# tusen-ai/MV2D

Hardware: AMD Instinct MI355X
Metric: multi-view samples/sec (6-cam frames) through the MV2D RoI-head hot path (higher is better)
Workload: dtype f16x3: every operand an fp16 hi + lo pair, three MFMAs per product, fp32 accumulation (fp32-class, index-exact route; the lo halves of the key / value rows are STORED as e4m3 bytes); 1 GPU; cfg2_s: MV2D-S head, 6 views 1408x512; global_batch=384, streams_per_gpu=4, samples_per_launch=16, pe_sine_branch=folded into a per-(weights, geometry) table, FLOPs not counted, parallelism=dp1, hipgraph=True

## Files before the change

mv2d_amd/csrc/xattn_fused.hip:

```cpp
#include "xattn_walk.h"
#include <stdlib.h>
#ifndef MV2D_XF_QB_DEFAULT
#define MV2D_XF_QB_DEFAULT 8
#endif

#ifdef MV2D_XF_TRACE
__device__ long long g_xf_trace[32];
#define XF_STAMP(i) do { if (blockIdx.x == MV2D_XF_TRACE && threadIdx.x == 0) g_xf_trace[i] = (long long)__builtin_amdgcn_s_memtime(); } while (0)
#else
#define XF_STAMP(i) do {} while (0)
#endif

namespace {

constexpr int WAVE_LDS = 16384;

template <int XLO, int QB>
__global__ __launch_bounds__(64 * QB, 2) void xattn_fused_kernel(const float* __restrict__ q, const uint4* __restrict__ WA_hi, const uint4* __restrict__ WA_lo,
                                                                const uint4* __restrict__ WB_hi, const uint4* __restrict__ WB_lo, const float* __restrict__ bv,
                                                                const unsigned short* __restrict__ Xk, const unsigned short* __restrict__ Xv,
                                                                const unsigned short* __restrict__ Xk_lo, const unsigned short* __restrict__ Xv_lo,
                                                                const int* __restrict__ row_ptr, const int* __restrict__ col_idx, float* __restrict__ ctx,
                                                                int R, int empty_nan, const int* __restrict__ order, int nblk) {
    constexpr int SMEM = QB * WAVE_LDS + QB * 512 + QB * HEADS * 4 + 3 * QB * 4;
    __shared__ __attribute__((aligned(16))) unsigned char smem[SMEM];
    const int tid = threadIdx.x, lane = tid & 63, wave = tid >> 6, n = lane & 15, g = lane >> 4;
    float* lsum = reinterpret_cast<float*>(smem + QB * WAVE_LDS + QB * 512);
    int* rq = reinterpret_cast<int*>(smem + QB * WAVE_LDS + QB * 512 + QB * HEADS * 4);
    int* rbeg = rq + QB;
    int* rend = rq + 2 * QB;
    const int blk = xcd_chunked(blockIdx.x, nblk);
    const int slot0 = (int)((long long)blk * R / nblk), nq = (int)((long long)(blk + 1) * R / nblk) - slot0;
    if (nq <= 0) return;
    XF_STAMP(0);
    if (tid < QB) {
        const int s = slot0 + min(tid, nq - 1);
        const int r_ = order ? order[s] : s;
        rq[tid] = r_;
        rbeg[tid] = row_ptr[r_];
        rend[tid] = row_ptr[r_ + 1];
    }
    __syncthreads();
    XF_STAMP(1);
    const int beg = rbeg[wave], end = rend[wave];
    const int ntile = wave < nq ? (end - beg + 15) >> 4 : 0;
    int idx_next = ntile > 0 ? col_idx[min(beg + n, end - 1)] : 0;
    typedef XattnWalk<XLO, false> Walk;
    Walk walk(Xk, Xv, Xk_lo, Xv_lo, lane, beg, end, reinterpret_cast<uint4*>(smem + wave * WAVE_LDS), reinterpret_cast<uint4*>(smem + wave * WAVE_LDS) + 512,
           reinterpret_cast<float*>(smem + QB * WAVE_LDS) + wave * 128);
    typename Walk::KRows k0;
    for (int h = wave; h < HEADS; h += QB) {
        const int r = rq[n & (QB - 1)];
        const float* qp = q + (long long)r * C + 32 * h + 8 * g;
        const float4 q0 = *reinterpret_cast<const float4*>(qp), q1 = *reinterpret_cast<const float4*>(qp + 4);
        const uint4* wh = WA_hi + (long long)h * 16 * 64 + lane;
        const uint4* wl = WA_lo + (long long)h * 16 * 64 + lane;
        uint4* qt = reinterpret_cast<uint4*>(smem + (n & (QB - 1)) * WAVE_LDS) + h * 64;
        u32x4 wa_h[16], wa_l[16];
#pragma unroll
        for (int t = 0; t < 16; ++t) {
            wa_h[t] = *reinterpret_cast<const u32x4*>(wh + t * 64);
            wa_l[t] = *reinterpret_cast<const u32x4*>(wl + t * 64);
        }
        __builtin_amdgcn_sched_barrier(0);
        XF_STAMP(20);
        Frag bh, bl;
        split8(q0, q1, bh, bl);
#pragma unroll
        for (int u = 0; u < 8; ++u) {
            if (u == 1) XF_STAMP(21);
            if (u == 4) XF_STAMP(22);
            f32x4_t a[2];
#pragma unroll
            for (int k = 0; k < 2; ++k) {
                f32x4_t c = {0.f, 0.f, 0.f, 0.f};
                c = mfma_q16_16x16x32(wa_l[2 * u + k], bh.v, c);
                c = mfma_q16_16x16x32(wa_h[2 * u + k], bl.v, c);
                c = mfma_q16_16x16x32(wa_h[2 * u + k], bh.v, c);
                a[k] = c;
            }
            Frag hi, lo;
            split8_k16(make_float4(a[0][0], a[0][1], a[0][2], a[0][3]), make_float4(a[1][0], a[1][1], a[1][2], a[1][3]), hi, lo);
            if (n < QB) {
                qt[u * 8 + g * 2] = hi.u;
                qt[u * 8 + g * 2 + 1] = lo.u;
            }
            if (u == (XLO ? 5 : 3) && h == wave && ntile > 0) walk.request_k(idx_next, k0);
        }
    }
    XF_STAMP(23);
    asm volatile("s_waitcnt lgkmcnt(0)" ::: "memory");
    __builtin_amdgcn_s_barrier();
    XF_STAMP(2);
    {
        const uint4* qp = reinterpret_cast<const uint4*>(smem + wave * WAVE_LDS) + (n & 7) * 64 + g * 2 + (n >> 3);
#pragma unroll
        for (int s = 0; s < 8; ++s) walk.qa[s].u = qp[s * 8];
    }
    walk.reset();
    if (ntile > 0) walk.stage_k(k0);
#pragma nounroll
    for (int tt = 0; tt < ntile; ++tt) {
        const int myidx = idx_next;
        if (tt + 1 < ntile) idx_next = col_idx[min(beg + 16 * (tt + 1) + n, end - 1)];
        typename Walk::VRows v;
        walk.gather(myidx, tt > 0, v);
        XF_STAMP(3 + 2 * min(tt, 5));
        walk.compute(tt, v);
        XF_STAMP(4 + 2 * min(tt, 5));
    }
    walk.row_sums();
    if (n == 0 && g < 2) {
#pragma unroll
        for (int i = 0; i < 4; ++i) lsum[wave * HEADS + 4 * g + i] = walk.l_run[i];
    }
    walk.store_z(reinterpret_cast<float*>(smem + wave * WAVE_LDS));
    XF_STAMP(15);
    __syncthreads();
    XF_STAMP(16);
    for (int h = wave; h < HEADS; h += QB) {
        const int j = n & (QB - 1);
        const float* zp = reinterpret_cast<const float*>(smem + j * WAVE_LDS) + h * C + 8 * g;
        const float rl = __builtin_amdgcn_rcpf(lsum[j * HEADS + h]);
        const uint4* wh = WB_hi + (long long)h * 16 * 64 + lane;
        const uint4* wl = WB_lo + (long long)h * 16 * 64 + lane;
        f32x4_t acc[2] = {{0.f, 0.f, 0.f, 0.f}, {0.f, 0.f, 0.f, 0.f}};
        u32x4 wb_h[16], wb_l[16];
#pragma unroll
        for (int t = 0; t < 16; ++t) {
            wb_h[t] = *reinterpret_cast<const u32x4*>(wh + t * 64);
            wb_l[t] = *reinterpret_cast<const u32x4*>(wl + t * 64);
        }
        int rr_[4], rp0_[4], rp1_[4];
#pragma unroll
        for (int i = 0; i < 4; ++i) {
            rr_[i] = rq[(4 * g + i) & (QB - 1)];
            rp0_[i] = rbeg[(4 * g + i) & (QB - 1)];
            rp1_[i] = rend[(4 * g + i) & (QB - 1)];
        }
        const float bv0 = bv[32 * h + n], bv1 = bv[32 * h + 16 + n];
        __builtin_amdgcn_sched_barrier(0);
#pragma unroll
        for (int s = 0; s < 8; ++s) {
            float4 x0 = *reinterpret_cast<const float4*>(zp + 32 * s);
            float4 x1 = *reinterpret_cast<const float4*>(zp + 32 * s + 4);
            x0 = make_float4(x0.x * rl, x0.y * rl, x0.z * rl, x0.w * rl);
            x1 = make_float4(x1.x * rl, x1.y * rl, x1.z * rl, x1.w * rl);
            Frag ah, al;
            split8(x0, x1, ah, al);
#pragma unroll
            for (int nt = 0; nt < 2; ++nt) {
                acc[nt] = mfma_q16_16x16x32(al.v, wb_h[s * 2 + nt], acc[nt]);
                acc[nt] = mfma_q16_16x16x32(ah.v, wb_l[s * 2 + nt], acc[nt]);
                acc[nt] = mfma_q16_16x16x32(ah.v, wb_h[s * 2 + nt], acc[nt]);
            }
        }
        if (4 * g < QB) {
#pragma unroll
            for (int i = 0; i < 4; ++i) {
                const int js = 4 * g + i;
                if (js < nq) {
                    const int rr = rr_[i];
                    const bool empty = rp1_[i] <= rp0_[i];
#pragma unroll
                    for (int nt = 0; nt < 2; ++nt) {
                        const int col = 32 * h + 16 * nt + n;
                        float v = acc[nt][i] + (nt ? bv1 : bv0);
                        if (empty) v = empty_nan ? __uint_as_float(0x7fc00000u) : 0.f;
                        ctx[(long long)rr * C + col] = v;
                    }
                }
            }
        }
    }
    XF_STAMP(17);
}

}

#ifdef MV2D_XF_TRACE
extern "C" int mv2d_xf_trace_read(long long* host, int n) { return hipMemcpyFromSymbol(host, HIP_SYMBOL(g_xf_trace), n * sizeof(long long)) == hipSuccess ? 0 : -2; }
#endif

extern "C" int mv2d_xattn_fused_fwd(const float* q, const void* WA_hi, const void* WA_lo, const void* WB_hi, const void* WB_lo, const float* bv,
                                    const void* Xk, const void* Xv, const void* Xk_lo, const void* Xv_lo, const int* row_ptr, const int* col_idx,
                                    float* ctx, int R, int empty_nan, const int* order, int lo_fmt, void* stream) {
    MV2D_CHECK_ARG(lo_fmt == 0 || (lo_fmt == 1 && Xk_lo), "mv2d_xattn_fused_fwd: lo_fmt is 0 (key16 lo rows) or 1 (e4m3 lo rows; needs the lo rows)");
    MV2D_CHECK_ARG(q && WA_hi && WA_lo && WB_hi && WB_lo && bv && Xk && Xv && row_ptr && col_idx && ctx && R >= 0, "mv2d_xattn_fused_fwd: bad args");
    MV2D_CHECK_ARG((Xk_lo == nullptr) == (Xv_lo == nullptr), "mv2d_xattn_fused_fwd: Xk_lo and Xv_lo come together");
    MV2D_CHECK_ARG(((uintptr_t)q & 15) == 0 && ((uintptr_t)WA_hi & 15) == 0 && ((uintptr_t)WA_lo & 15) == 0 && ((uintptr_t)WB_hi & 15) == 0 &&
                       ((uintptr_t)WB_lo & 15) == 0 && ((uintptr_t)Xk & 15) == 0 && ((uintptr_t)Xv & 15) == 0 && ((uintptr_t)Xk_lo & 15) == 0 &&
                       ((uintptr_t)Xv_lo & 15) == 0, "mv2d_xattn_fused_fwd: operands must be 16-byte aligned");
    if (R == 0) return MV2D_OK;
    static int n_cu = 0;
    if (n_cu == 0) {
        hipDeviceProp_t prop;
        int dev = 0;
        n_cu = (hipGetDevice(&dev) == hipSuccess && hipGetDeviceProperties(&prop, dev) == hipSuccess && prop.multiProcessorCount > 0) ? prop.multiProcessorCount : 256;
    }
    static const int qb_env = [] { const char* e = getenv("MV2D_XF_QB"); return e ? atoi(e) : 0; }();
    const int QB = qb_env == 4 || qb_env == 8 ? qb_env : MV2D_XF_QB_DEFAULT;
    const int slots = n_cu * (QB == 4 ? 2 : 1);
    int nblk = (R + QB - 1) / QB;
    if (nblk > slots) {
        const int up = (nblk + slots - 1) / slots * slots;
        if ((long long)up * (QB / 2) <= R) nblk = up;
    } else {
        const int spread = R / 2 < n_cu ? R / 2 : n_cu;
        if (spread > nblk) nblk = spread;
    }
    const dim3 grid(nblk), block(64 * QB);
#define MV2D_XF(XLO_, QB_) hipLaunchKernelGGL((xattn_fused_kernel<XLO_, QB_>), grid, block, 0, (hipStream_t)stream, q, (const uint4*)WA_hi, (const uint4*)WA_lo, \
                                              (const uint4*)WB_hi, (const uint4*)WB_lo, bv, (const unsigned short*)Xk, (const unsigned short*)Xv,                     \
                                              (const unsigned short*)Xk_lo, (const unsigned short*)Xv_lo, row_ptr, col_idx, ctx, R, empty_nan, order, nblk)
    if (Xk_lo && lo_fmt == 1) { if (QB == 4) MV2D_XF(2, 4); else MV2D_XF(2, 8); }
    else if (Xk_lo) { if (QB == 4) MV2D_XF(1, 4); else MV2D_XF(1, 8); }
    else { if (QB == 4) MV2D_XF(0, 4); else MV2D_XF(0, 8); }
#undef MV2D_XF
    MV2D_LAUNCH_CHECK();
    return MV2D_OK;
}
```

mv2d_amd/csrc/xattn_walk.h:

```cpp
#pragma once
#include "common.h"
#include <type_traits>

namespace {

constexpr int C = 256, HEADS = 8;
constexpr float LOG2E = 1.4426950408889634f;

typedef q16x8_t q16x8;
union Frag { uint4 u; q16x8 v; };
typedef unsigned int u32x4 __attribute__((ext_vector_type(4)));
typedef unsigned int u32x2 __attribute__((ext_vector_type(2)));

__device__ __forceinline__ void split8(const float4& x0, const float4& x1, Frag& hi, Frag& lo) {
    const float f[8] = {x0.x, x0.y, x0.z, x0.w, x1.x, x1.y, x1.z, x1.w};
    unsigned int h[4], l[4];
#pragma unroll
    for (int i = 0; i < 4; ++i) split_q16x2(f[2 * i], f[2 * i + 1], h[i], l[i]);
    hi.u = make_uint4(h[0], h[1], h[2], h[3]);
    lo.u = make_uint4(l[0], l[1], l[2], l[3]);
}
__device__ __forceinline__ void split8_k16(const float4& x0, const float4& x1, Frag& hi, Frag& lo) {
    const float f[8] = {x0.x, x0.y, x0.z, x0.w, x1.x, x1.y, x1.z, x1.w};
    unsigned int h[4], l[4];
#pragma unroll
    for (int i = 0; i < 4; ++i) split_k16x2(f[2 * i], f[2 * i + 1], h[i], l[i]);
    hi.u = make_uint4(h[0], h[1], h[2], h[3]);
    lo.u = make_uint4(l[0], l[1], l[2], l[3]);
}

__device__ __forceinline__ unsigned int lo_pair(unsigned int a, unsigned int b) { return __builtin_amdgcn_perm(b, a, 0x05040100u); }
__device__ __forceinline__ unsigned int hi_pair(unsigned int a, unsigned int b) { return __builtin_amdgcn_perm(b, a, 0x07060302u); }

#define XATTN_DPP(v, ctrl) __uint_as_float((unsigned)__builtin_amdgcn_update_dpp(0, (int)__float_as_uint(v), ctrl, 0xF, 0xF, true))
__device__ __forceinline__ float row16_max(float v) {
    v = fmaxf(v, XATTN_DPP(v, 0xB1));
    v = fmaxf(v, XATTN_DPP(v, 0x4E));
    v = fmaxf(v, XATTN_DPP(v, 0x141));
    v = fmaxf(v, XATTN_DPP(v, 0x140));
    return v;
}

template <int XLO, bool DBG>
struct XattnWalk {
    typedef std::conditional_t<XLO == 2, u32x2, u32x4> lo_t;
    struct KRows { u32x4 hi[8]; lo_t lo[XLO ? 8 : 1]; };
    struct VRows { u32x4 hi[4][2]; lo_t lo[XLO ? 4 : 1][2]; };

    const unsigned short *Xk, *Xv, *Xk_lo, *Xv_lo;
    int lane, n, g, beg, end;
    uint4 *kt, *kt2;
    float* pl;
    float* dbg_logits;
    long long dbg_stride;
    Frag qa[8];
    float m_run[4], l_run[4];
    f32x4_t Z[16];

    __device__ __forceinline__ XattnWalk(const unsigned short* Xk_, const unsigned short* Xv_, const unsigned short* Xk_lo_, const unsigned short* Xv_lo_,
                                         int lane_, int beg_, int end_, uint4* kt_, uint4* kt2_, float* pl_, float* dbg_logits_ = nullptr,
                                         long long dbg_stride_ = 0)
        : Xk(Xk_), Xv(Xv_), Xk_lo(Xk_lo_), Xv_lo(Xv_lo_), lane(lane_), n(lane_ & 15), g(lane_ >> 4), beg(beg_), end(end_), kt(kt_), kt2(kt2_), pl(pl_),
          dbg_logits(dbg_logits_), dbg_stride(dbg_stride_) {}

    __device__ __forceinline__ void reset() {
#pragma unroll
        for (int i = 0; i < 4; ++i) { m_run[i] = -INFINITY; l_run[i] = 0.f; }
#pragma unroll
        for (int u = 0; u < 16; ++u) Z[u] = f32x4_t{0.f, 0.f, 0.f, 0.f};
    }

    __device__ __forceinline__ void load_v(const unsigned short* V_, int myidx, u32x4 (&dst)[4][2]) const {
#pragma unroll
        for (int e = 0; e < 4; ++e) {
            const unsigned int vidx = (unsigned int)__shfl(myidx, 4 * g + e, 64);
            const char* vp = reinterpret_cast<const char*>(V_) + ((vidx << 9) + 16u * (unsigned)n);
            dst[e][0] = *reinterpret_cast<const u32x4*>(vp);
            dst[e][1] = *reinterpret_cast<const u32x4*>(vp + 256);
        }
    }
    __device__ __forceinline__ void load_k(const unsigned short* K_, int myidx, u32x4 (&dst)[8]) const {
#pragma unroll
        for (int i = 0; i < 8; ++i) {
            const unsigned int ridx = (unsigned int)__shfl(myidx, 2 * i + (lane >> 5), 64);
            dst[i] = *reinterpret_cast<const u32x4*>(reinterpret_cast<const char*>(K_) + ((ridx << 9) + (unsigned)(lane & 31) * 16u));
        }
    }
    __device__ __forceinline__ void store_k(uint4* tile, const u32x4 (&src)[8]) const {
#pragma unroll
        for (int i = 0; i < 8; ++i) {
            const int rowi = 2 * i + (lane >> 5);
            reinterpret_cast<u32x4*>(tile)[rowi * 32 + ((lane & 31) ^ (rowi & 15))] = src[i];
        }
    }
    __device__ __forceinline__ void load_v8(const unsigned short* V_, int myidx, u32x2 (&dst)[4][2]) const {
#pragma unroll
        for (int e = 0; e < 4; ++e) {
            const unsigned int vidx = (unsigned int)__shfl(myidx, 4 * g + e, 64);
            const char* vp = reinterpret_cast<const char*>(V_) + ((vidx << 8) + 8u * (unsigned)n);
            dst[e][0] = *reinterpret_cast<const u32x2*>(vp);
            dst[e][1] = *reinterpret_cast<const u32x2*>(vp + 128);
        }
    }
    __device__ __forceinline__ void load_k8(const unsigned short* K_, int myidx, u32x2 (&dst)[8]) const {
#pragma unroll
        for (int i = 0; i < 8; ++i) {
            const unsigned int ridx = (unsigned int)__shfl(myidx, 2 * i + (lane >> 5), 64);
            dst[i] = *reinterpret_cast<const u32x2*>(reinterpret_cast<const char*>(K_) + ((ridx << 8) + (unsigned)(lane & 31) * 8u));
        }
    }
    __device__ __forceinline__ void store_k8(uint4* tile, const u32x2 (&src)[8]) const {
#pragma unroll
        for (int i = 0; i < 8; ++i) {
            const int rowi = 2 * i + (lane >> 5);
            tile[rowi * 32 + ((lane & 31) ^ (rowi & 15))] = lo8_chunk(make_uint2(src[i].x, src[i].y));
        }
    }
    __device__ __forceinline__ void request_k(int myidx, KRows& k) const {
        load_k(Xk, myidx, k.hi);
        if constexpr (XLO == 1) load_k(Xk_lo, myidx, k.lo);
        if constexpr (XLO == 2) load_k8(Xk_lo, myidx, k.lo);
    }
    __device__ __forceinline__ void stage_k(const KRows& k) const {
        store_k(kt, k.hi);
        if constexpr (XLO == 1) store_k(kt2, k.lo);
        if constexpr (XLO == 2) store_k8(kt2, k.lo);
    }
    __device__ __forceinline__ void request_v(int myidx, VRows& v) const {
        load_v(Xv, myidx, v.hi);
        if constexpr (XLO == 1) load_v(Xv_lo, myidx, v.lo);
        if constexpr (XLO == 2) load_v8(Xv_lo, myidx, v.lo);
    }

    __device__ __forceinline__ void gather(int myidx, bool with_k, VRows& v) const {
        if constexpr (XLO != 0) {
            if (with_k) {
                KRows k;
                request_k(myidx, k);
                stage_k(k);
            }
            request_v(myidx, v);
        } else if (with_k) {
            KRows k;
            request_k(myidx, k);
            request_v(myidx, v);
            stage_k(k);
        } else {
            request_v(myidx, v);
        }
        __builtin_amdgcn_wave_barrier();
    }

    __device__ __forceinline__ void compute(int tt, const VRows& v) {
        const int kbase = beg + 16 * tt;
        f32x4_t sacc = {0.f, 0.f, 0.f, 0.f};
#pragma unroll
        for (int s = 0; s < 8; ++s) {
            Frag kb;
            kb.u = kt[n * 32 + ((4 * s + g) ^ n)];
            sacc = mfma_k16_16x16x32(qa[s].u, kb.u, sacc);
            if (XLO) {
                Frag kl, qh;
                kl.u = kt2[n * 32 + ((4 * s + g) ^ n)];
                qh.u = n < 8 ? qa[s].u : make_uint4(0u, 0u, 0u, 0u);
                sacc = mfma_k16_16x16x32(qh.u, kl.u, sacc);
            }
        }
        const bool valid = kbase + n < end;
        float sv[4], p[4], alpha[4];
#pragma unroll
        for (int i = 0; i < 4; ++i) {
            const auto sw = __builtin_amdgcn_permlane32_swap(__float_as_uint(sacc[i]), __float_as_uint(sacc[i]), false, false);
            const float full = __uint_as_float(sw[0]) + __uint_as_float(sw[1]);
            if (DBG && dbg_logits && g < 2 && valid) dbg_logits[(long long)(4 * g + i) * dbg_stride + kbase + n] = full;
            sv[i] = valid ? full * LOG2E : -INFINITY;
        }
#pragma unroll
        for (int i = 0; i < 4; ++i) {
            float tm = sv[i];
            tm = row16_max(tm);
            const float m_new = fmaxf(m_run[i], tm);
            alpha[i] = __builtin_amdgcn_exp2f(m_run[i] - m_new);
            p[i] = __builtin_amdgcn_exp2f(sv[i] - m_new);
            l_run[i] = l_run[i] * alpha[i] + p[i];
            m_run[i] = m_new;
        }
        if (g < 2) {
#pragma unroll
            for (int i = 0; i < 4; ++i) pl[(4 * g + i) * 16 + n] = p[i];
        }
        __builtin_amdgcn_wave_barrier();
        uint2 pa, pah;
        {
            const float4 pv = *reinterpret_cast<const float4*>(pl + (n & 7) * 16 + 4 * g);
            unsigned int h0, h1, l0, l1;
            split_k16x2_bounded(pv.x, pv.y, h0, l0);
            split_k16x2_bounded(pv.z, pv.w, h1, l1);
            pa = n < 8 ? make_uint2(h0, h1) : make_uint2(l0, l1);
            pah = n < 8 ? make_uint2(h0, h1) : make_uint2(0u, 0u);
        }
#pragma unroll
        for (int u = 0; u < 16; ++u)
#pragma unroll
            for (int i = 0; i < 4; ++i) Z[u][i] *= alpha[i];
#pragma unroll
        for (int H = 0; H < 2; ++H) {
            const unsigned int r0[4] = {v.hi[0][H].x, v.hi[0][H].y, v.hi[0][H].z, v.hi[0][H].w};
            const unsigned int r1[4] = {v.hi[1][H].x, v.hi[1][H].y, v.hi[1][H].z, v.hi[1][H].w};
            const unsigned int r2[4] = {v.hi[2][H].x, v.hi[2][H].y, v.hi[2][H].z, v.hi[2][H].w};
            const unsigned int r3[4] = {v.hi[3][H].x, v.hi[3][H].y, v.hi[3][H].z, v.hi[3][H].w};
#pragma unroll
            for (int w = 0; w < 8; ++w) {
                const int d = w >> 1;
                const uint2 vb = (w & 1) ? make_uint2(hi_pair(r0[d], r1[d]), hi_pair(r2[d], r3[d]))
                                         : make_uint2(lo_pair(r0[d], r1[d]), lo_pair(r2[d], r3[d]));
                f32x4_t zc = Z[H * 8 + w];
                zc = mfma_k16_16x16x16(pa, vb, zc);
                if constexpr (XLO != 0) {
                    auto lo_pair_of = [&](int e) -> unsigned int {
                        if constexpr (XLO == 2) {
                            const unsigned int b = v.lo[e][H][d >> 1];
                            return (d & 1) ? lo8_pair<1>(b) : lo8_pair<0>(b);
                        } else {
                            return v.lo[e][H][d];
                        }
                    };
                    const unsigned int q0 = lo_pair_of(0), q1 = lo_pair_of(1), q2 = lo_pair_of(2), q3 = lo_pair_of(3);
                    const uint2 vl = (w & 1) ? make_uint2(hi_pair(q0, q1), hi_pair(q2, q3)) : make_uint2(lo_pair(q0, q1), lo_pair(q2, q3));
                    zc = mfma_k16_16x16x16(pah, vl, zc);
                }
                Z[H * 8 + w] = zc;
            }
        }
        __builtin_amdgcn_wave_barrier();
    }

    __device__ __forceinline__ void row_sums() {
#pragma unroll
        for (int i = 0; i < 4; ++i) {
            float l = l_run[i];
            l += __shfl_xor(l, 1, 64);
            l += __shfl_xor(l, 2, 64);
            l += __shfl_xor(l, 4, 64);
            l += __shfl_xor(l, 8, 64);
            l_run[i] = l;
        }
    }
    __device__ __forceinline__ void store_z(float* szw) const {
#pragma unroll
        for (int H = 0; H < 2; ++H)
#pragma unroll
            for (int i = 0; i < 4; ++i) {
                float v[4];
#pragma unroll
                for (int w = 0; w < 4; ++w) {
                    const auto sw = __builtin_amdgcn_permlane32_swap(__float_as_uint(Z[H * 8 + w][i]), __float_as_uint(Z[H * 8 + w + 4][i]), false, false);
                    v[w] = __uint_as_float(sw[0]) + __uint_as_float(sw[1]);
                }
                float* dst = szw + (4 * (g & 1) + i) * C + 128 * H + 8 * n + 4 * (g >> 1);
                *reinterpret_cast<float4*>(dst) = make_float4(v[0], v[1], v[2], v[3]);
            }
    }
};

}
```

Measured before the change: 8812 samples/s.

## Prefetch short tail tile rows early and hoist first output-projection weight load

```diff
diff --git a/mv2d_amd/csrc/xattn_fused.hip b/mv2d_amd/csrc/xattn_fused.hip
--- a/mv2d_amd/csrc/xattn_fused.hip
+++ b/mv2d_amd/csrc/xattn_fused.hip
@@ -2,6 +2,15 @@
 #include <stdlib.h>
 #ifndef MV2D_XF_QB_DEFAULT
 #define MV2D_XF_QB_DEFAULT 8
+#endif
+#ifndef MV2D_XF_TAIL
+#define MV2D_XF_TAIL 1
+#endif
+#ifndef MV2D_XF_HOIST_C
+#define MV2D_XF_HOIST_C 1
+#endif
+#ifndef MV2D_XF_ROUNDS
+#define MV2D_XF_ROUNDS 1
 #endif
 
 #ifdef MV2D_XF_TRACE
@@ -45,7 +54,7 @@
     const int beg = rbeg[wave], end = rend[wave];
     const int ntile = wave < nq ? (end - beg + 15) >> 4 : 0;
     int idx_next = ntile > 0 ? col_idx[min(beg + n, end - 1)] : 0;
-    typedef XattnWalk<XLO, false> Walk;
+    typedef XattnWalk<XLO, false, MV2D_XF_TAIL> Walk;
     Walk walk(Xk, Xv, Xk_lo, Xv_lo, lane, beg, end, reinterpret_cast<uint4*>(smem + wave * WAVE_LDS), reinterpret_cast<uint4*>(smem + wave * WAVE_LDS) + 512,
            reinterpret_cast<float*>(smem + QB * WAVE_LDS) + wave * 128);
     typename Walk::KRows k0;
@@ -98,17 +107,35 @@
         for (int s = 0; s < 8; ++s) walk.qa[s].u = qp[s * 8];
     }
     walk.reset();
+    const int tail_tile = (ntile >= 2 && end - beg - 16 * (ntile - 1) <= MV2D_XF_TAIL) ? ntile - 1 : -1;
+    typename Walk::TailRows tail;
     if (ntile > 0) walk.stage_k(k0);
 #pragma nounroll
     for (int tt = 0; tt < ntile; ++tt) {
         const int myidx = idx_next;
         if (tt + 1 < ntile) idx_next = col_idx[min(beg + 16 * (tt + 1) + n, end - 1)];
         typename Walk::VRows v;
-        walk.gather(myidx, tt > 0, v);
+        if (MV2D_XF_TAIL > 0 && tt == tail_tile) {
+            walk.fill_tail(tail, v);
+        } else {
+            walk.gather(myidx, tt > 0, v);
+            if (MV2D_XF_TAIL > 0 && tt + 1 == tail_tile) walk.request_tail(idx_next, tail);
+        }
         XF_STAMP(3 + 2 * min(tt, 5));
         walk.compute(tt, v);
         XF_STAMP(4 + 2 * min(tt, 5));
     }
+    u32x4 wb_h[16], wb_l[16];
+    if (MV2D_XF_HOIST_C) {
+        const uint4* wh = WB_hi + (long long)wave * 16 * 64 + lane;
+        const uint4* wl = WB_lo + (long long)wave * 16 * 64 + lane;
+#pragma unroll
+        for (int t = 0; t < 16; ++t) {
+            wb_h[t] = *reinterpret_cast<const u32x4*>(wh + t * 64);
+            wb_l[t] = *reinterpret_cast<const u32x4*>(wl + t * 64);
+        }
+        __builtin_amdgcn_sched_barrier(0);
+    }
     walk.row_sums();
     if (n == 0 && g < 2) {
 #pragma unroll
@@ -116,20 +143,28 @@
     }
     walk.store_z(reinterpret_cast<float*>(smem + wave * WAVE_LDS));
     XF_STAMP(15);
-    __syncthreads();
+    if (MV2D_XF_HOIST_C) {
+        asm volatile("s_waitcnt lgkmcnt(0)" ::: "memory");
+        __builtin_amdgcn_s_barrier();
+    } else {
+        __syncthreads();
+    }
     XF_STAMP(16);
-    for (int h = wave; h < HEADS; h += QB) {
+#pragma unroll
+    for (int hh = 0; hh < HEADS / QB; ++hh) {
+        const int h = wave + hh * QB;
         const int j = n & (QB - 1);
         const float* zp = reinterpret_cast<const float*>(smem + j * WAVE_LDS) + h * C + 8 * g;
         const float rl = __builtin_amdgcn_rcpf(lsum[j * HEADS + h]);
         const uint4* wh = WB_hi + (long long)h * 16 * 64 + lane;
         const uint4* wl = WB_lo + (long long)h * 16 * 64 + lane;
         f32x4_t acc[2] = {{0.f, 0.f, 0.f, 0.f}, {0.f, 0.f, 0.f, 0.f}};
-        u32x4 wb_h[16], wb_l[16];
-#pragma unroll
-        for (int t = 0; t < 16; ++t) {
-            wb_h[t] = *reinterpret_cast<const u32x4*>(wh + t * 64);
-            wb_l[t] = *reinterpret_cast<const u32x4*>(wl + t * 64);
+        if (!MV2D_XF_HOIST_C || hh > 0) {
+#pragma unroll
+            for (int t = 0; t < 16; ++t) {
+                wb_h[t] = *reinterpret_cast<const u32x4*>(wh + t * 64);
+                wb_l[t] = *reinterpret_cast<const u32x4*>(wl + t * 64);
+            }
         }
         int rr_[4], rp0_[4], rp1_[4];
 #pragma unroll
@@ -202,10 +237,10 @@
     const int QB = qb_env == 4 || qb_env == 8 ? qb_env : MV2D_XF_QB_DEFAULT;
     const int slots = n_cu * (QB == 4 ? 2 : 1);
     int nblk = (R + QB - 1) / QB;
-    if (nblk > slots) {
+    if (nblk > slots && MV2D_XF_ROUNDS) {
         const int up = (nblk + slots - 1) / slots * slots;
         if ((long long)up * (QB / 2) <= R) nblk = up;
-    } else {
+    } else if (nblk <= slots) {
         const int spread = R / 2 < n_cu ? R / 2 : n_cu;
         if (spread > nblk) nblk = spread;
     }
diff --git a/mv2d_amd/csrc/xattn_walk.h b/mv2d_amd/csrc/xattn_walk.h
--- a/mv2d_amd/csrc/xattn_walk.h
+++ b/mv2d_amd/csrc/xattn_walk.h
@@ -41,11 +41,12 @@
     return v;
 }
 
-template <int XLO, bool DBG>
+template <int XLO, bool DBG, int TAIL = 0>
 struct XattnWalk {
     typedef std::conditional_t<XLO == 2, u32x2, u32x4> lo_t;
     struct KRows { u32x4 hi[8]; lo_t lo[XLO ? 8 : 1]; };
     struct VRows { u32x4 hi[4][2]; lo_t lo[XLO ? 4 : 1][2]; };
+    struct TailRows { u32x4 k_hi[TAIL ? TAIL : 1]; lo_t k_lo[TAIL ? TAIL : 1]; u32x4 v_hi[TAIL ? TAIL : 1][2]; lo_t v_lo[TAIL ? TAIL : 1][2]; };
 
     const unsigned short *Xk, *Xv, *Xk_lo, *Xv_lo;
     int lane, n, g, beg, end;
@@ -147,6 +148,61 @@
             stage_k(k);
         } else {
             request_v(myidx, v);
+        }
+        __builtin_amdgcn_wave_barrier();
+    }
+
+    __device__ __forceinline__ void request_tail(int idx_last, TailRows& t) const {
+#pragma unroll
+        for (int j = 0; j < TAIL; ++j) {
+            const unsigned int idx = (unsigned int)__shfl(idx_last, j, 64);
+            t.k_hi[j] = *reinterpret_cast<const u32x4*>(reinterpret_cast<const char*>(Xk) + ((idx << 9) + (unsigned)(lane & 31) * 16u));
+            if constexpr (XLO == 1) t.k_lo[j] = *reinterpret_cast<const u32x4*>(reinterpret_cast<const char*>(Xk_lo) + ((idx << 9) + (unsigned)(lane & 31) * 16u));
+            if constexpr (XLO == 2) t.k_lo[j] = *reinterpret_cast<const u32x2*>(reinterpret_cast<const char*>(Xk_lo) + ((idx << 8) + (unsigned)(lane & 31) * 8u));
+        }
+#pragma unroll
+        for (int j = 0; j < TAIL; ++j) {
+            const unsigned int idx = (unsigned int)__shfl(idx_last, j, 64);
+            const char* vp = reinterpret_cast<const char*>(Xv) + ((idx << 9) + 16u * (unsigned)n);
+            t.v_hi[j][0] = *reinterpret_cast<const u32x4*>(vp);
+            t.v_hi[j][1] = *reinterpret_cast<const u32x4*>(vp + 256);
+            if constexpr (XLO == 1) {
+                const char* lp = reinterpret_cast<const char*>(Xv_lo) + ((idx << 9) + 16u * (unsigned)n);
+                t.v_lo[j][0] = *reinterpret_cast<const u32x4*>(lp);
+                t.v_lo[j][1] = *reinterpret_cast<const u32x4*>(lp + 256);
+            }
+            if constexpr (XLO == 2) {
+                const char* lp = reinterpret_cast<const char*>(Xv_lo) + ((idx << 8) + 8u * (unsigned)n);
+                t.v_lo[j][0] = *reinterpret_cast<const u32x2*>(lp);
+                t.v_lo[j][1] = *reinterpret_cast<const u32x2*>(lp + 128);
+            }
+        }
+    }
+    __device__ __forceinline__ void fill_tail(const TailRows& t, VRows& v) const {
+        static_assert(TAIL <= 4, "the value rows of the held keys belong to lanes g == 0");
+        const bool odd = lane >= 32;
+#pragma unroll
+        for (int i = 0; i < 8; ++i) {
+            const int rowi = 2 * i + (lane >> 5);
+            const int at = rowi * 32 + ((lane & 31) ^ (rowi & 15));
+            constexpr int T1 = TAIL ? TAIL - 1 : 0;
+            const int j0 = 2 * i < T1 ? 2 * i : T1, j1 = 2 * i + 1 < T1 ? 2 * i + 1 : T1;
+            reinterpret_cast<u32x4*>(kt)[at] = (j0 != j1 && odd) ? t.k_hi[j1] : t.k_hi[j0];
+            if constexpr (XLO == 1) reinterpret_cast<u32x4*>(kt2)[at] = (j0 != j1 && odd) ? t.k_lo[j1] : t.k_lo[j0];
+            if constexpr (XLO == 2) {
+                const lo_t lo = (j0 != j1 && odd) ? t.k_lo[j1] : t.k_lo[j0];
+                kt2[at] = lo8_chunk(make_uint2(lo.x, lo.y));
+            }
+        }
+#pragma unroll
+        for (int e = 0; e < 4; ++e) {
+            constexpr int T1 = TAIL ? TAIL - 1 : 0;
+            const int j = e < T1 ? e : T1;
+#pragma unroll
+            for (int H = 0; H < 2; ++H) {
+                v.hi[e][H] = (j != T1 && g == 0) ? t.v_hi[j][H] : t.v_hi[T1][H];
+                if constexpr (XLO != 0) v.lo[e][H] = (j != T1 && g == 0) ? t.v_lo[j][H] : t.v_lo[T1][H];
+            }
         }
         __builtin_amdgcn_wave_barrier();
     }
```

Measured after the change: 8848 samples/s, median of 6. About the same (+0.4%).
